# social-ai-uoft/sorrel

Measured on AMD Instinct MI355X. Metric: agent-steps/sec, higher is better.
Workload: dtype u8 grid, f32 obs

## Files before the change

### sorrel_amd/csrc/common.h

```cpp
#pragma once


constexpr int kBlock = 256;
constexpr int kWave = 64;
constexpr int kMaxPass = 2;

struct DevTables {
    uint32_t thr_lo[SGW_MAX_TYPES];
    uint32_t delta[4][SGW_MAX_TYPES];
    double value[SGW_MAX_TYPES];
    uint8_t spawn_choice[SGW_MAX_TYPES][SGW_MAX_CHOICES];
    uint8_t spawn_count[SGW_MAX_TYPES];
    uint8_t agent_type[SGW_MAX_AGENTS];
    uint8_t dense_choice[SGW_MAX_CHOICES];
    uint8_t layer_fill[8];
    uint8_t layer_border[8];
    uint8_t pad_[8];
    uint8_t rule[SGW_MAX_TYPES];
    int8_t rule_layer[SGW_MAX_TYPES];
    uint8_t rule_become[SGW_MAX_TYPES];
    uint8_t pad2_[SGW_MAX_TYPES];
    uint32_t rule_mask[SGW_MAX_TYPES];
    uint32_t delta3[SGW_MAX_TYPES];
    double appearance[SGW_MAX_TYPES][SGW_MAX_CHANNELS];
// ... 58 lines not shown
    uint32_t first_env;
    int64_t E;
    uint32_t epoch, turn, flags;
    int a0, a1;
    int do_move;
    int obs_post;
    int obs_u8;
    int agent_rule;
    uint32_t tag_it, tag_notit;
    double tag_reward;
    uint8_t* agent_state;
    uint8_t* agent_dir;
    int has_become;
    uint32_t quiet0, quiet1;
    uint32_t kind_pack;
    int beam_radius;
    uint32_t clean_beam, zap_beam, beam_block_mask;
    int total_factor;
    uint8_t* state_at_pov;
    uint64_t dense_thr;
    int dense_count;
    uint8_t* grid;
    uint8_t* pos;
    uint8_t* actions;
    float* obs;
    float* rewards;
    double* total;
    const DevTables* tab;
    const uint8_t* tmpl;
    int* status;
    int obs_stage;
    int stage_agents;
    int obs_next;
    int obs_A, obs_a0;
    int64_t obs_ag;
    int big_pitch;
    int big_stage;
    int big_stage_off;
    uint32_t* walk_ctr;
    int walk_word;
    int walk_static;
    int single_spawner;
    int rows_mode;
    int rows_by_agent;
    int onehot;
    int tail_kind, tail_len;
    const float* tail_table;
    const TurnState* ts;
    uint32_t nturns;
    int64_t ts_obs, ts_act, ts_rew;
    uint32_t extras;
    uint32_t drawn_mask;
    uint8_t* target_types;
};
constexpr uint32_t kExtraDrawn = 1u, kExtraTargets = 2u;
#ifdef SGW_JIT
constexpr bool kExtrasDefault = false;
#else
constexpr bool kExtrasDefault = true;
#endif
constexpr bool extras_default_tables(const int tc) { return kExtrasDefault && tc == 0; }
template <bool XTRAS>
__device__ __forceinline__ uint32_t extras_of(const Params& p) {
    if constexpr (XTRAS) return p.extras;
    else return 0u;
}

struct U4 {
    uint32_t x, y, z, w;
};

__device__ __forceinline__ uint32_t xor3(uint32_t a, uint32_t b, uint32_t k) {
    uint32_t d;
    asm("v_bitop3_b32 %0, %1, %2, %3 bitop3:0x96" : "=v"(d) : "v"(a), "v"(b), "s"(k));
    return d;
}

template <bool OWN_KEYS = true>
__device__ __forceinline__ U4 philox4x32_10(uint32_t c0, uint32_t c1, uint32_t c2, uint32_t c3,
                                            uint32_t k0, uint32_t k1) {
#ifndef SGW_DIAG_SHARED_KEYS
    if constexpr (OWN_KEYS) asm volatile("" : "+s"(k0), "+s"(k1));
#endif
#pragma unroll
    for (int r = 0; r < 10; ++r) {
        const uint64_t p0 = (uint64_t)0xD2511F53u * c0;
        const uint64_t p1 = (uint64_t)0xCD9E8D57u * c2;
        const uint32_t n0 = xor3((uint32_t)(p1 >> 32), c1, k0);
        const uint32_t n2 = xor3((uint32_t)(p0 >> 32), c3, k1);
        c1 = (uint32_t)p1;
        c3 = (uint32_t)p0;
        c0 = n0;
        c2 = n2;
        k0 += 0x9E3779B9u;
        k1 += 0xBB67AE85u;
    }
    return U4{c0, c1, c2, c3};
}

__device__ __forceinline__ uint32_t opaque(uint32_t v) {
    asm volatile("" : "+v"(v));
    return v;
}

struct PhiloxUniform {
    uint32_t r1_n2;
    uint32_t r2_n0;
    uint32_t r2_n2;
    uint32_t r3_n2;
};
__device__ __forceinline__ PhiloxUniform philox_uniform(const uint32_t c1, const uint32_t c2, const uint32_t c3, const uint32_t k0, const uint32_t k1) {
    const uint64_t p1 = (uint64_t)0xCD9E8D57u * c2;
    const uint32_t n0 = (uint32_t)(p1 >> 32) ^ c1 ^ k0;
    const uint64_t q0 = (uint64_t)0xD2511F53u * n0;
    PhiloxUniform u;
    u.r1_n2 = opaque(c3 ^ k1);
    u.r2_n0 = opaque((uint32_t)p1 ^ (k0 + 0x9E3779B9u));
    u.r2_n2 = opaque((uint32_t)(q0 >> 32) ^ (k1 + 0xBB67AE85u));
// ... 300 lines not shown
```

### sorrel_amd/csrc/plan.h

```cpp
#pragma once

struct Kernel {
    const void* host = nullptr;
    const char* host_name = "-";
    std::string want;
    bool x_twin = false;
    bool compile_time_tables = false;
    hipFunction_t jit = nullptr;
    hipFunction_t jit_x = nullptr;
    bool tried_x = false;
    bool tried = false;
    bool usable() const { return host != nullptr || !want.empty(); }
    const char* name() const { return (jit || (!host && !want.empty())) ? want.c_str() : host_name; }
};

uint64_t prob_threshold(double pr) {
    const double t = std::floor(pr * 4294967296.0);
    if (!(t > 0.0)) return 0;
    if (t >= 4294967296.0) return 4294967296ull;
    return (uint64_t)t;
}

int validate(const sgw_config* c) {
    if (!c) return fail(SGW_EINVAL, "config is NULL");
// ... 514 lines not shown
    p.fill_delta3 = h.delta3[c.fill_type];
    p.fill_delta16[0] = h.delta16[0][c.fill_type];
    p.fill_delta16[1] = h.delta16[1][c.fill_type];
    int& nspawn = w.nspawn;
    p.spawn_pat = 0xFFFFFFFFu;
    for (int t = 0; t < c.num_types; ++t) {
        if (c.type_rule[t] != SGW_RULE_SPAWN) continue;
        ++nspawn;
        p.spawn_pat = 0x01010101u * (uint32_t)t;
        const uint64_t thr = prob_threshold(c.spawn_prob[t]);
        p.spawn_thr = (uint32_t)(thr & 0xFFFFFFFFull);
        p.spawn_full = thr >= 4294967296ull ? 1u : 0u;
        p.spawn_n = c.spawn_count[t];
        p.choice_lo = p.choice_hi = 0;
        for (int k = 0; k < c.spawn_count[t]; ++k) {
            if (k < 4) p.choice_lo |= (uint32_t)c.spawn_choice[t][k] << (8 * k);
            else p.choice_hi |= (uint32_t)c.spawn_choice[t][k] << (8 * (k - 4));
        }
    }
    p.single_spawner = nspawn <= 1 ? 1 : 0;
    p.onehot = onehot ? 1 : 0;
    p.nturns = 1;
    p.obs_A = c.num_agents;
    p.obs_a0 = 0;
    p.seed_lo = (uint32_t)c.seed;
    p.seed_hi = (uint32_t)(c.seed >> 32);
    p.first_env = (uint32_t)c.first_env_id;
    p.E = c.num_envs;
    p.dense_thr = prob_threshold(c.dense_prob);
    p.dense_count = c.dense_count;
    p.obs_post = c.obs_post;
    p.agent_rule = c.agent_rule;
    p.tag_it = c.tag_it_type;
    p.tag_notit = c.tag_notit_type;
    p.tag_reward = c.tag_reward;
    p.agent_mask = 0;
    for (int a = 0; a < c.num_agents; ++a) p.agent_mask |= 1u << (c.agent_type[a] & 31u);
    if (c.agent_rule == SGW_AGENT_RULE_TAG) p.agent_mask |= (1u << (c.tag_it_type & 31u)) | (1u << (c.tag_notit_type & 31u));
    p.has_become = 0;
    p.become_mask = 0;
    for (int t = 0; t < c.num_types; ++t)
        if (c.type_rule[t] == SGW_RULE_BECOME_IF) {
            p.has_become = 1;
            p.become_mask |= 1u << t;
        }
    p.quiet0 = p.quiet1 = 0xFFFFFFFFu;
    for (int z = 0; z < c.layers; ++z) {
        const uint32_t t = c.layer_fill_type[z];
        if (t >= (uint32_t)c.num_types || c.type_rule[t] != SGW_RULE_NONE) continue;
        const uint32_t w = 0x01010101u * t;
        if (p.quiet0 == 0xFFFFFFFFu || p.quiet0 == w) p.quiet0 = w;
        else if (p.quiet1 == 0xFFFFFFFFu || p.quiet1 == w) p.quiet1 = w;
    }
    p.kind_pack = 0;
    for (int a = 0; a < c.num_actions; ++a) p.kind_pack |= (uint32_t)(c.action_kind[a] & 3u) << (2 * a);
    p.beam_radius = c.beam_radius;
    p.clean_beam = c.clean_beam_type;
    p.zap_beam = c.zap_beam_type;
    p.beam_block_mask = c.beam_block_mask;
    p.total_factor = c.reward_total_factor > 0 ? c.reward_total_factor : 1;
}

void plan_family(Planning& w, Plan* e) {
    PLANNING_INPUTS;
    const int nspawn = w.nspawn;
    const bool plain_move = c.agent_rule == SGW_AGENT_RULE_MOVE;
    const bool tagk = c.agent_rule == SGW_AGENT_RULE_TAG;
    const bool simple_rules = !p.has_become && c.agent_rule != SGW_AGENT_RULE_CLEANUP;
    const bool vec16 = (p.env_stride & 15) == 0 && p.env_stride >= p.cells_pad;
    const int rules_units = (c.num_envs >= 16384 || o.rules_11k) ? kMaxUnitsPlain : kMaxUnitsRules;
    bool rules_8k = !simple_rules && !tagk && vec16 && p.cells_pad > 4096 && (p.cells_pad >> 4) <= 64 * rules_units && p.VV <= 128;
    if (!o.fast_rules || o.force_generic) rules_8k = false;
    const bool fast_8k_ok = simple_rules && (onehot || (e->rgb16 && c.num_channels == 3)) && vec16 && nspawn <= 1 && p.cells_pad > 4096 && (p.cells_pad >> 4) <= 64 * kMaxUnitsPlain && p.VV <= 128;
    bool fast_8k = fast_8k_ok && c.num_envs >= (p.cells_pad <= 8192 ? 4096 : 16384);
    if (o.fast_8k == 0) fast_8k = false;
    if (o.fast_8k == 1) fast_8k = fast_8k_ok;
    if (o.force_generic) fast_8k = false;
    e->wpe = (p.cells_pad <= 4096 || rules_8k || fast_8k) ? 1 : 4;
    if (o.force_big && simple_rules && !o.force_generic) e->wpe = 4;
    const bool many_agents = c.num_agents > 64;
    if (many_agents) e->wpe = 4;
    const int epb = kBlock / (e->wpe * kWave);
    e->lds_bytes = (size_t)p.tab_bytes + (size_t)epb * p.env_lds;
    e->fast = e->wpe == 1 && vec16 && (p.cells_pad >> 4) <= 64 * (fast_8k ? kMaxUnitsPlain : kMaxUnits) && nspawn <= 1 && p.VV <= 128 && simple_rules;
    e->fast_rules = !e->fast && e->wpe == 1 && vec16 && (p.cells_pad >> 4) <= 64 * rules_units && p.VV <= 128 &&
                    !tagk && (p.cells_pad <= 4096 || rules_8k);
    if (!o.fast_rules) e->fast_rules = false;
    e->fast = e->fast || e->fast_rules;
    if (many_agents) e->fast = e->fast_rules = false;
    const bool rgb16_fast = e->rgb16 && e->fast && !e->fast_rules && c.num_channels == 3;
    const bool bytes_ok = onehot || rgb16_fast;
    e->fast_tab_bytes = bytes_ok ? 4 * SGW_MAX_TYPES * 4 : SGW_MAX_TYPES * SGW_MAX_CHANNELS * 8;
    bool agents_impassable = true;
    for (int a = 0; a < c.num_agents; ++a) agents_impassable = agents_impassable && !c.type_passable[c.agent_type[a]];
    const bool tag_move = tagk;
    e->big = e->wpe == 4 && vec16 && nspawn <= 1 && p.VV <= 128 && agents_impassable && (plain_move || tag_move) && simple_rules && !many_agents;
    e->big_threads = kBigThreads;
    if (e->big) e->big_threads = big_threads_for(o, onehot, c.num_agents, p.VV);
    w.plain_move = plain_move; w.tagk = tagk; w.many_agents = many_agents; w.fast_8k = fast_8k; w.epb = epb;
    w.rgb16_fast = rgb16_fast; w.bytes_ok = bytes_ok;
}

void plan_obs_staging(Planning& w, Plan* e) {
    PLANNING_INPUTS;
    const bool tagk = w.tagk, fast_8k = w.fast_8k, bytes_ok = w.bytes_ok;
    bool stage_kernel = false;
// ... 128 lines not shown
    if (e->whole_env_burst && static_map && !e->fast_rules && ((C * (2 * r + 1) * (2 * r + 1)) & 1) == 0) {
        if (L == 2 && C == 6 && r == 3 && H == 32 && W == 32 && !tagk) {
            e->k_sweep_rows.host = reinterpret_cast<const void*>(&step_fast_rows<2, 6, 3, 32, 32>);
            e->k_sweep_rows.host_name = "step_fast_rows<2, 6, 3, 32, 32>";
        }
        if (jit) e->k_sweep_rows.want = fast_rows_id(L, C, r, H, W, tagk);
        if (jit) e->k_sweep_rows_tail.want = fast_rows_id(L, C, r, H, W, tagk, true);
    }
    if (jit && !e->whole_env_burst && stage_kernel && e->onehot && !e->rgb16 && e->stage_agents >= 1) {
        e->k_sweep_rows.want = step.d.shaped(L, C, r, jh, jw).rowsx_id();
        e->sweep_rows_chunked = !e->k_sweep_rows.want.empty();
    }
}
void plan_instances(Planning& w, Plan* e) {
    PLANNING_INPUTS;
    const bool tagk = w.tagk, many_agents = w.many_agents;
    const bool tag_move = tagk;
    const int L = c.layers, C = c.num_channels, r = c.vision_radius, H = c.height, W = c.width;
    for (Kernel* k : {&e->k_step, &e->k_plain, &e->k_multi, &e->k_walk}) k->x_twin = true;
    e->k_sweep_rows.x_twin = !e->fast;
    if (e->fast) {
        plan_fast_instances(w, e);
    } else if (e->big) {
        set_prebuilt(e->k_step, pick_big(e->onehot, L, C, r, tag_move, e->big_threads));
        if (!tag_move) set_prebuilt(e->k_multi, pick_big_multi(e->onehot, L, C, r));
        if (!tag_move && ((p.cells + 15) >> 4) <= 4 * e->big_threads)
            set_prebuilt(e->k_walk, pick_big_walk(e->onehot, L, C, r, e->big_threads));
        if (jit) {
            e->k_sweep_rows.want = big_id(e->onehot, L, C, r, false, false, tag_move, e->big_threads, true);
            e->k_step.want = big_id(e->onehot, L, C, r, false, false, tag_move, e->big_threads);
            if (!tag_move) e->k_multi.want = big_id(e->onehot, L, C, r, true, false, false, kBigThreads);
            if (e->k_walk.host) e->k_walk.want = big_id(e->onehot, L, C, r, false, true, false, e->big_threads);
        }
    } else {
        if (many_agents) {
            e->k_step.host = pick_step_many(e->onehot, c.agent_rule, false, &e->k_step.host_name);
            e->k_multi.host = nullptr;
        } else {
            e->k_step.host = pick_step(o, e->group, e->onehot, L, C, c.agent_rule, r, H, W, false, &e->k_step.host_name);
            e->k_multi.host = pick_step(o, e->group, e->onehot, L, C, c.agent_rule, r, H, W, true, &e->k_multi.host_name);
        }
        if (jit) {
            e->k_step.want = generic_id(e->group, e->onehot, L, C, c.agent_rule, r, H, W, false, many_agents);
            e->k_multi.want = generic_id(e->group, e->onehot, L, C, c.agent_rule, r, H, W, true, many_agents);
            e->k_sweep_rows.want = generic_id(e->group, e->onehot, L, C, c.agent_rule, r, H, W, false, many_agents, true);
        }
    }
    if (!o.big_walk) e->k_walk = Kernel();
    for_each_kernel(*e, kHasPrebuiltTwin, [](Kernel& k) {
        if (k.host && k.want == k.host_name) k.want.clear();
        return 0;
    });
    e->multi_turn = e->k_multi.usable();
}

void plan_row_kernels(Planning& w, Plan* e) {
    PLANNING_INPUTS;
    const bool plain_move = w.plain_move;
    const int L = c.layers, C = c.num_channels, r = c.vision_radius;
    e->reset_fn = pick_reset(e->wpe);
    e->phase_ok = plain_move && e->wpe == 4;
    if (o.phase_kernel >= 0) e->phase_ok = plain_move && o.phase_kernel == 1;
    if (e->onehot && p.cells >= 8 && o.phase_rows) {
        const int NW = (C + 3) / 4;
        e->k_rows.x_twin = true;
        e->k_rows.host = pick_rows(L, NW, r, &e->k_rows.host_name, &e->k_obs_rows.host, &e->k_obs_rows.host_name);
        if (jit && !e->k_rows.host && r >= 1 && r <= 7) {
            e->k_rows.want = rows_id("phase_rows", L, NW, r);
            e->k_obs_rows.want = rows_id("observe_rows", L, NW, r);
        }
        if (!plain_move) e->k_rows = Kernel();
        if (e->k_obs_rows.usable()) {
            const int V = 2 * r + 1;
            e->rows_epb = e->rows_wpb = 4 * (64 / (V <= 4 ? 4 : (V <= 8 ? 8 : 16)));
            e->rows_lds = (size_t)4 * (NW * 34 * 4 + SGW_MAX_TYPES * 8 + (((e->rows_epb / 4) * C * V * V + 15) & ~15));
        }
    }
}

void plan_geometry(Planning& w, Plan* e) {
    PLANNING_INPUTS;
    const int epb = w.epb, epb_step = w.epb_step;
    p.stage_agents = e->stage_agents;
    if (o.fast_wg_per_cu > 0) { e->fast_wg_cap = o.fast_wg_per_cu; e->fast_wg_cap_forced = true; }
    e->grid_blocks = (int)ceil_div(p.E, (e->fast || e->big) ? epb : epb_step);
    if (e->k_walk.usable()) {
        const size_t walk_lds = e->step_lds_bytes - (size_t)(e->big_threads / 64) * e->big_stage;
        const int per_cu = resident_per_cu(e->big_threads, walk_lds, SGW_WALK_WAVES);
        const int plain_per_cu = resident_per_cu(e->big_threads, e->step_lds_bytes, SGW_BIG_WAVES);
        e->walk_blocks = per_cu * w.num_cus;
        e->walk_min_envs = (int64_t)plain_per_cu * w.num_cus * 3 / 2;
        e->walk_max_envs = e->big_stage ? (int64_t)plain_per_cu * w.num_cus * 9 / 4 : (int64_t)plain_per_cu * w.num_cus * 3;
        if (o.big_walk_blocks > 0) {
            e->walk_blocks = o.big_walk_blocks;
            e->walk_min_envs = e->walk_blocks;
            e->walk_max_envs = INT64_MAX;
        }
    }
    if (e->big) {
        const int64_t by_lds = (int64_t)(kLdsPerCu / (((e->step_lds_bytes + 1023) & ~(size_t)1023) + 1024));
        const int64_t resident = std::max<int64_t>(1, std::min<int64_t>(2048 / e->big_threads, by_lds));
        e->big_stage_min_envs = resident * w.num_cus * 7 / 4;
        if (o.big_stage == 1) e->big_stage_min_envs = 0;
    }
    e->reset_blocks = (int)ceil_div(p.E, epb);
}
// ... 21 lines not shown
```

### sorrel_amd/csrc/sgw.hip

```cpp
#include <hip/hip_runtime.h>
#include <hip/hiprtc.h>

#include <dlfcn.h>
#include <fcntl.h>
#include <sys/stat.h>
#include <unistd.h>

#include <algorithm>
#include <chrono>
#include <cmath>
#include <cstdarg>
#include <cstdio>
#include <cstdlib>
#include <cstring>
#include <mutex>
#include <new>
#include <string>
#include <unordered_map>
#include <vector>

#include "../../include/sgw.h"

namespace {

// ... 1299 lines not shown
    *launches = e->launches;
    e->ms_acc = 0.0;
    e->launches = 0;
    return SGW_OK;
}

int sgw_get_step_times_ms(sgw_engine* e, float* out_ms, int64_t capacity, int64_t* count) {
    if (!e || !count || (capacity > 0 && !out_ms)) return fail(SGW_EINVAL, "sgw_get_step_times_ms: NULL argument");
    if (int rc = time_drain(e)) return rc;
    const int64_t n = std::min<int64_t>((int64_t)e->series.size(), std::max<int64_t>(capacity, 0));
    for (int64_t i = 0; i < n; ++i) out_ms[i] = e->series[(size_t)i];
    const int64_t lost = (int64_t)e->series.size() - n + e->series_dropped;
    *count = n;
    e->series.clear();
    e->series_dropped = 0;
    if (lost > 0) {
        fail(SGW_OK, "sgw_get_step_times_ms: %lld launches not returned (capacity %lld, series cap %lld)", (long long)lost,
             (long long)capacity, (long long)kSeriesCap);
        return 1;
    }
    return SGW_OK;
}

int sgw_set_auto_reset(sgw_engine* e, uint32_t max_turns, double* episode_return) {
    if (!e) return fail(SGW_EINVAL, "sgw_set_auto_reset: NULL engine");
    e->auto_max_turns = max_turns;
    e->episode_return = max_turns ? episode_return : nullptr;
    return SGW_OK;
}

int sgw_set_wg_per_cu(sgw_engine* e, int wg_per_cu) {
    if (!e) return fail(SGW_EINVAL, "sgw_set_wg_per_cu: NULL engine");
    if (wg_per_cu < -1 || wg_per_cu > 8) return fail(SGW_EINVAL, "wg_per_cu must be -1 (never cap), 0 (automatic) or 1..8");
    e->wg_per_cu = wg_per_cu;
    return SGW_OK;
}

int sgw_launch_info(sgw_engine* e, char* buf, int64_t capacity) {
    if (!e || !buf || capacity < 1) return fail(SGW_EINVAL, "sgw_launch_info: NULL argument");
    Params p = e->base;
    p.a0 = 0; p.a1 = p.A; p.flags = SGW_STEP_SWEEP | SGW_STEP_RANDOM_ACTIONS; p.do_move = 1;
    p.obs = reinterpret_cast<float*>(16); p.obs_u8 = e->obs_format == SGW_OBS_U8 ? 1 : 0;
    StepLaunch d;
    if (int rc = step_launch(e, p, nullptr, &d)) return rc;
    Kernel& k = *d.k;
    if (d.walk) (void)resolve_kernel(e, k);
    int per_cu = 0;
    hipError_t oe = k.jit ? hipModuleOccupancyMaxActiveBlocksPerMultiprocessor(&per_cu, k.jit, (int)d.threads, d.lds_info)
                          : (k.host ? hipOccupancyMaxActiveBlocksPerMultiprocessor(&per_cu, k.host, (int)d.threads, d.lds_info) : hipErrorInvalidValue);
    if (oe != hipSuccess) per_cu = -1;
    const char* phase = e->k_rows.usable() ? e->k_rows.name() : (e->phase_ok ? (e->onehot ? "phase_kernel<true>" : "phase_kernel<false>") : "the step kernel");
    const char* srows = e->k_sweep_rows.usable() ? ((e->tail_kind != SGW_TAIL_NONE && e->fast && !e->sweep_rows_chunked && e->k_sweep_rows_tail.jit) ? e->k_sweep_rows_tail.name()
                                                                                                                                                   : e->k_sweep_rows.name()) : "-";
    snprintf(buf, (size_t)capacity, "%s group=%d threads=%d lds=%zu env_lds=%d obs_stage=%d stage_agents=%d grid=%d wg_per_cu=%d cap=%s%d phase=%s big_stage=%d specialised=%d sweep_rows=%s",
             k.name(),
             (e->fast || e->big) ? (e->big ? e->big_threads : e->wpe * kWave) : e->group,
             (int)d.threads, d.lds_info, e->step_env_lds, e->obs_stage, e->stage_agents,
             (int)d.blocks, per_cu,
             e->wg_per_cu == 0 ? "auto:" : (e->wg_per_cu < 0 ? "never:" : "forced:"), d.cap, phase, d.big_stage,
             k.jit ? 1 : 0, srows);
    return SGW_OK;
}

}
```

### sorrel_amd/csrc/step_fast.h

```cpp
#pragma once

constexpr int kMaxUnits = 4;
constexpr int kMaxUnitsRules = 8;
constexpr int kMaxUnitsPlain = 11;
constexpr size_t kLdsPerCu = 160 * 1024;
constexpr size_t kCacheResidentGrid = (size_t)288 << 20;

#define OBS_STORE(ptr, val) (*(ptr) = (val))


template <class Draw>
__device__ __forceinline__ uint32_t sweep_hits_with(const uint4& u, const Params& p, Draw draw) {
    uint32_t hits = 0;
    const uint32_t pat = p.spawn_pat & 0xFFu;
#pragma unroll
    for (int k = 0; k < 4; ++k) {
        const uint32_t dv = k == 0 ? u.x : k == 1 ? u.y : k == 2 ? u.z : u.w;
        const bool m0 = (dv & 0xFFu) == pat, m1 = ((dv >> 8) & 0xFFu) == pat, m2 = ((dv >> 16) & 0xFFu) == pat, m3 = (dv >> 24) == pat;
        if (m0 | m1 | m2 | m3) {
            const U4 w = draw(k);
            const bool f = p.spawn_full != 0;
            uint32_t hb = 0;
            hb |= (m0 && (f || w.x < p.spawn_thr)) ? 1u : 0u;
            hb |= (m1 && (f || w.y < p.spawn_thr)) ? 2u : 0u;
// ... 258 lines not shown
    const uint32_t vt_lo = (uint32_t)__double_as_longlong(vtab), vt_hi = (uint32_t)(__double_as_longlong(vtab) >> 32);
    const uint32_t vt_f32 = __float_as_uint((float)vtab);
    const bool write_obs = !(p.flags & SGW_STEP_NO_OBS);
    const bool do_sweep = (p.flags & SGW_STEP_SWEEP) != 0;
    const bool dirty = do_sweep || (p.do_move && p.a1 > p.a0);
    const bool sweep_only = !RULES && (MULTI ? p.nturns : 1u) == 1u && !(p.do_move && p.a1 > p.a0);

    {
        double tot = p.do_move ? p.total[env] : 0.0;

#ifdef SGW_STAMPS
        asm volatile("s_waitcnt vmcnt(0)" ::: "memory");
#endif
        STAMP(1);
        [[maybe_unused]] uint32_t hits[NU];
        if constexpr (!kStatic || ((TL * TH * TW) & 15) != 0) {
            if (cells & 15) {
#pragma unroll
                for (int k = 0; k < NU; ++k)
                    if (lane + 64 * k == nunits - 1) {
                        const int tail = cells & 15;
                        uint32_t d[4] = {u[k].x, u[k].y, u[k].z, u[k].w};
#pragma unroll
                        for (int q = 0; q < 4; ++q) {
                            const int keep = tail - 4 * q;
                            if (keep <= 0) d[q] = 0xFFFFFFFFu;
                            else if (keep < 4) d[q] |= 0xFFFFFFFFu << (8 * keep);
                        }
                        u[k] = make_uint4(d[0], d[1], d[2], d[3]);
                    }
            }
        }
#pragma unroll
        for (int k = 0; k < NU; ++k)
            if (lane + 64 * k < nunits) lg16[lane + 64 * k] = u[k];
        if constexpr (RULES || !kStatic) {
            const uint4* src = reinterpret_cast<const uint4*>(p.grid + env * p.env_stride);
            for (int i = 64 * NU + lane; i < nunits; i += 64) {
                uint4 v = src[i];
                if ((cells & 15) && i == nunits - 1) {
                    const int tail = cells & 15;
                    uint32_t d[4] = {v.x, v.y, v.z, v.w};
#pragma unroll
                    for (int q = 0; q < 4; ++q) {
                        const int keep = tail - 4 * q;
                        if (keep <= 0) d[q] = 0xFFFFFFFFu;
                        else if (keep < 4) d[q] |= 0xFFFFFFFFu << (8 * keep);
                    }
                    v = make_uint4(d[0], d[1], d[2], d[3]);
                }
                lg16[i] = v;
            }
        }
        int st_lane = 0;
        uint32_t taddr_v = 0xFFFFFFFFu, oaddr_v = 0, npos = 0, rew_bits = 0, moved = 0;
        const uint32_t nturns = MULTI ? p.nturns : 1u;
        for (uint32_t tix = 0; tix < nturns; ++tix) {
        const uint32_t turn = turn0 + tix;
        constexpr uint32_t kNotDrawn = 0xFFFFFFFFu;
        if (rnd) act = kNotDrawn;
        if constexpr (RULES) {
            gsync<1>();
            if (do_sweep) {
                sweep_ordered<1, 64>(p, rt, lg, env_id, lane, turn, ep4, L, HW);
            }
        } else if constexpr (!kStatic) {
            gsync<1>();
            if (do_sweep) {
                sweep_single<64>(p, lg, env_id, lane, turn, ep4,
                                 sweep_only ? reinterpret_cast<uint32_t*>(p.grid + env * p.env_stride) : nullptr);
                gsync<1>();
            }
        } else {
            if (tix > 0) {
                gsync<1>();
#pragma unroll
                for (int k = 0; k < NU; ++k)
                    if (lane + 64 * k < nunits) u[k] = lg16[lane + 64 * k];
            }
            const PhiloxUniform pu = philox_uniform(turn, env_id, ep4 | SGW_STREAM_SPAWN, p.seed_lo, p.seed_hi);
#pragma unroll
            for (int k = 0; k < NU; ++k) {
                hits[k] = 0;
                if ((k < kFullRounds || !kTailDword) && lane + 64 * k < nunits && do_sweep)
                    hits[k] = sweep_hits<kOwnKeys>(u[k], (uint32_t)(lane + 64 * k), p, pu);
            }
            gsync<1>();
            if (do_sweep) {
                typedef typename HitMask<(NU > 2)>::type hm_t;
                static_assert(NU <= 4, "16 hit bits per unit, four units per lane");
                hm_t hm = 0;
#pragma unroll
                for (int k = 0; k < NU; ++k) hm |= (hm_t)hits[k] << (16 * k);
                auto unit_off = [&](const uint32_t b) { return ((uint32_t)lane + 64u * (b >> 4)) * 16u + (b & 15u); };
                auto kind_of = [&](const uint32_t pick) { return (uint8_t)(((pick < 4 ? p.choice_lo : p.choice_hi) >> (8 * (pick & 3u))) & 0xFFu); };
                uint32_t nlist = 0;
                bool fused = false;
                if constexpr (!ROWS && !MULTI) {
                    uint32_t fl = p.flags;
                    asm("" : "+s"(fl));
                    if (stage && !(fl & SGW_STEP_NO_OBS) && p.do_move && rnd && p.a0 == 0 && p.a1 == p.A && p.obs_stage >= 256) {
                        uint16_t* list = reinterpret_cast<uint16_t*>(ob);
                        const uint32_t room = 64u - (uint32_t)p.A;
                        hm_t rest = hm;
                        uint64_t m = __ballot(rest != 0);
                        while (m != 0 && nlist <= room) {
// ... 104 lines not shown
            const int i0 = (lo + 3) >> 2, i1 = he >> 2;
            const int ie = lane == 0 ? i0 - 1 : i1;
            const bool edge = lane == 0 ? (lo & 3) != 0 : (lane == 1 && (he & 3) != 0 && (i1 >= i0 || (lo & 3) == 0));
            if (ROWX || !p.obs_u8) {
                float* gb = ROWX ? row_dst - sh : p.obs + (e0 - sh);
                burst_emit<true>(gb, i0, i1, lane, [&](const int i) { return ob4[i]; }, tof);
                if (edge) {
                    const uint32_t b = ob4[ie];
#pragma unroll
                    for (int j = 0; j < 4; ++j)
                        if (4 * ie + j >= lo && 4 * ie + j < he) gb[4 * ie + j] = tof((b >> (8 * j)) & 0xFFu);
                }
            } else {
                uint8_t* gb = reinterpret_cast<uint8_t*>(p.obs) + (e0 - sh);
                burst_emit<false>(gb, i0, i1, lane, [&](const int i) { return ob4[i]; }, tof);
                if (edge) {
                    const uint32_t b = ob4[ie];
#pragma unroll
                    for (int j = 0; j < 4; ++j)
                        if (4 * ie + j >= lo && 4 * ie + j < he) gb[4 * ie + j] = (uint8_t)(b >> (8 * j));
                }
            }
            if constexpr (ROWX) {
                if (p.tail_kind != SGW_TAIL_NONE) {
                    float* t = row_dst + C * VV;
                    if (p.tail_kind == SGW_TAIL_AGENT_IS_IT) {
                        const uint32_t ty_ = (uint32_t)__builtin_amdgcn_readlane((int)atype, a_lo);
                        if (lane == 0) t[0] = ty_ == p.tag_it ? 1.f : 0.f;
                    } else {
                        const int ay_ = __builtin_amdgcn_readlane((int)(yx & 0xFFu), a_lo), ax_ = __builtin_amdgcn_readlane((int)(yx >> 8), a_lo);
                        const float* src = p.tail_table + ((int64_t)ay_ * W + ax_) * p.tail_len;
                        for (int k = lane; k < p.tail_len; k += 64) t[k] = src[k];
                    }
                }
            }
            if (!last) {
                uint8_t t = 0;
                if (lane < hi - he) t = ob[he + lane];
                gsync<1>();
                if (lane < hi - he) ob[lane] = t;
                ch_shift = (uint32_t)(hi - he);
                ch_lo = 0;
            }
            gsync<1>();
        };
        [[maybe_unused]] uint32_t fill_v[NW];
        constexpr bool kFillRegs = ONEHOT && kStatic && !RULES && !STAGE && !P3 && !I16;
        if constexpr (kFillRegs) {
#pragma unroll
            for (int q = 0; q < NW; ++q) fill_v[q] = opaque(p.fill_delta[q]);
        }
        constexpr bool kVersioned = ONEHOT && kStatic && !kStageAlways && !TAG && !RULES && !ROWS && !MULTI;
        const bool lean = kVersioned && stage && write_obs && !p.obs_next;
        auto window = [&](const int a, const int y, const int x, const int s_o, auto lean_c) {
            constexpr bool LEAN = decltype(lean_c)::value;
            {
                const int cbase = s_o - zoff;
                int a_s = a;
                if constexpr (kVersioned && !LEAN) asm volatile("" : "+s"(a_s));
                [[maybe_unused]] float* obase = p.obs + turn_obs + ((env * p.obs_A + (a_s - p.obs_a0)) * (int64_t)C) * VV;
#pragma unroll
                for (int k = 0; k < 2; ++k) {
                    if (64 * k >= VV) break;
                    const int w = lane + 64 * k;
                    if (w < VV) {
#ifdef SGW_DIAG_SKIP_GATHER
                        if (p.turn != 0xFFFFFFFFu) continue;
#endif
                        const bool inb = (unsigned)(y + wdi[k]) < (unsigned)H && (unsigned)(x + wdj[k]) < (unsigned)W;
                        const int off = inb ? cbase + woff[k] : 0;
                        [[maybe_unused]] float* o = obase + w;
                        if constexpr (ONEHOT) {
                            uint32_t cnt[NW];
#pragma unroll
                            for (int q = 0; q < NW; ++q) cnt[q] = 0;
#pragma unroll
                            for (int z = 0; z < (TL ? TL : 1); ++z) {
                                const uint32_t t = lg[z * HW + off] & 31u;
#pragma unroll
                                for (int q = 0; q < NW; ++q) cnt[q] += wdelta[q * 32 + t];
                            }
                            if constexpr (TL == 0) {
                                for (int z = 1; z < L; ++z) {
                                    const uint32_t t = lg[z * HW + off] & 31u;
#pragma unroll
                                    for (int q = 0; q < NW; ++q) cnt[q] += wdelta[q * 32 + t];
                                }
                            }
#pragma unroll
                            for (int q = 0; q < NW; ++q) cnt[q] = inb ? cnt[q] : (kFillRegs ? fill_v[q] : P3 ? p.fill_delta3 : I16 ? p.fill_delta16[q] : p.fill_delta[q]);
                            auto chan = [&](const int c) -> uint32_t {
                                if constexpr (P3) return (cnt[0] >> (3 * c)) & 7u;
                                else if constexpr (I16) return min((cnt[c >> 1] >> (16 * (c & 1))) & 0xFFFFu, 255u);
                                else return (cnt[c >> 2] >> (8 * (c & 3))) & 0xFFu;
                            };
                            if (LEAN || stage) {
                                uint8_t* os = ob + (kStageAlways ? (int)ch_shift + ((a - ch_a0) * C) * VV : (a * C) * VV) + w;
                                if constexpr (TC != 0) {
#pragma unroll
                                    for (int c = 0; c < CMAX; ++c)
                                        if (c < C) os[c * VV] = (uint8_t)chan(c);
                                } else {
#pragma unroll
                                    for (int g = 0; g < (CMAX + 3) / 4; ++g)
                                        if (4 * g < C) {
#pragma unroll
                                            for (int b = 0; b < 4; ++b)
                                                if (4 * g + b < CMAX) os[(4 * g + b) * VV] = (uint8_t)chan(4 * g + b);
                                        }
                                }
                            } else if constexpr (kStageAlways) {
                            } else if (!p.obs_u8) {
#pragma unroll
                                for (int c = 0; c < CMAX; ++c)
                                    if (c < C) OBS_STORE(o + c * VV, tof(chan(c)));
                            } else {
                                uint8_t* o8 = reinterpret_cast<uint8_t*>(p.obs) + (o - p.obs);
#pragma unroll
                                for (int c = 0; c < CMAX; ++c)
                                    if (c < C) o8[c * VV] = (uint8_t)chan(c);
                            }
                        } else {
                            for (int c = 0; c < C; ++c) {
                                double acc = wapp[lg[off] & 31u][c];
                                for (int z = 1; z < L; ++z) acc += wapp[lg[z * HW + off] & 31u][c];
                                OBS_STORE(o + c * VV, obs_finish(inb ? acc : wapp[p.fill_type][c], p.obs_post));
                            }
                        }
                    }
                }
            }
        };
        const int a_end = (p.obs_next && p.a1 < p.A) ? p.a1 + 1 : p.a1;
        for (int a = p.a0; a < a_end; ++a) {
            if constexpr (ROWX) {
                if (a > p.a0 && write_obs) emit_chunk(a - 1, a, true);
                ch_a0 = a;
                row_dst = static_cast<float*>(rp->p[a]) + env * rp->stride;
                ch_lo = ch_shift = (uint32_t)(reinterpret_cast<uintptr_t>(row_dst) >> 2) & kLineMask;
            } else if constexpr (kStageAlways) {
                if (a - ch_a0 == p.stage_agents) {
                    if (write_obs) emit_chunk(ch_a0, a, false);
                    ch_a0 = a;
                }
            }
            const uint32_t yx_a = (uint32_t)__builtin_amdgcn_readlane((int)yx, a);
            const int y = (int)(yx_a & 0xFFu), x = (int)(yx_a >> 8);
            const int s_o = zoff + y * W + x;
            if (lean) {
                if constexpr (kVersioned) window(a, y, x, s_o, BoolC<true>{});
            } else if (p.obs_next ? a == p.a1 : write_obs) {
                window(a, y, x, s_o, BoolC<false>{});
            }
            if (!p.do_move || a >= p.a1) continue;
            const uint32_t s_t = (uint32_t)__builtin_amdgcn_readlane((int)taddr_v, a);
            const uint32_t my_type = (uint32_t)__builtin_amdgcn_readlane((int)atype, a);
            const bool valid = s_t != 0xFFFFFFFFu;
            if constexpr (RULES) {
                if (p.agent_rule == SGW_AGENT_RULE_CLEANUP) {
                    const uint32_t kd = (uint32_t)__builtin_amdgcn_readlane((int)kind_v, a);
                    const uint32_t kind = kd & 3u, ndir = kd >> 4;
                    const bool aok = (kd & 4u) != 0;
                    const uint32_t facing = (uint32_t)__builtin_amdgcn_readlane((int)adir, a) & 3u;
                    const int ay = __builtin_amdgcn_readlane((int)py, a), ax = __builtin_amdgcn_readlane((int)px, a);
                    if (aok && kind != SGW_ACTION_MOVE && p.zA + 1 < L) {
                        if (lane < 3 * p.beam_radius) {
                            const int arm = lane / p.beam_radius, i = lane - arm * p.beam_radius;
                            const int fy = facing == 0 ? -1 : facing == 2 ? 1 : 0, fx = facing == 1 ? 1 : facing == 3 ? -1 : 0;
                            const int ry = facing == 1 ? 1 : facing == 3 ? -1 : 0, rx = facing == 0 ? 1 : facing == 2 ? -1 : 0;
                            const int step = arm == 0 ? i + 1 : i, side = arm == 0 ? 0 : (arm == 1 ? 1 : -1);
                            const int by = ay + side * ry + step * fy, bx = ax + side * rx + step * fx;
                            if ((unsigned)by < (unsigned)H && (unsigned)bx < (unsigned)W) {
                                const int boff = (p.zA + 1) * HW + by * W + bx;
                                if (!((p.beam_block_mask >> (lg[boff] & 31u)) & 1u))
                                    lg[boff] = (uint8_t)(kind == SGW_ACTION_CLEAN ? p.clean_beam : p.zap_beam);
                            }
                        }
                        gsync<1>();
                    }
                    double val = 0.0;
                    uint32_t t = 0xFFu;
                    if (valid) {
                        const int tc = (int)s_t - zoff;
                        for (int zl = 0; zl < L; ++zl) {
                            const uint32_t tz = (uint32_t)__builtin_amdgcn_readfirstlane((int)lg[zl * HW + tc]) & 31u;
                            const uint32_t lo_ = (uint32_t)__builtin_amdgcn_readlane((int)vt_lo, (int)tz);
                            const uint32_t hi_ = (uint32_t)__builtin_amdgcn_readlane((int)vt_hi, (int)tz);
                            val += __longlong_as_double(((long long)hi_ << 32) | lo_);
                        }
                        t = (uint32_t)__builtin_amdgcn_readfirstlane((int)lg[s_t]);
                    }
                    const bool pass = valid && t < (uint32_t)p.T && ((p.pass_mask >> (t & 31u)) & 1u);
                    if (pass && lane == 0) {
                        lg[s_t] = (uint8_t)my_type;
                        lg[s_o] = (uint8_t)p.default_type;
                    }
                    moved = lane == a ? (pass ? 1u : 0u) : moved;
                    adir = (lane == a && aok && kind == SGW_ACTION_MOVE && ndir < 4u) ? ndir : adir;
                    rew_bits = lane == a ? __float_as_uint((float)val) : rew_bits;
                    tot += val * (double)(p.total_factor - 1);
                    tot += val;
                    gsync<1>();
                    continue;
                }
            }
            const uint32_t t = (uint32_t)__builtin_amdgcn_readfirstlane((int)lg[valid ? s_t : (uint32_t)s_o]);
// ... 171 lines not shown
```

Measured before the change: 4.766 billion.

## Skip gathering inert uniform layers in onehot observation window

At plan time, layers whose fill type never changes, is never spawned, and contributes zero to every observation channel are marked inert. In the kernel, each wave checks via ballot whether such a layer is still uniformly filled and, if so, skips that layer's per-cell lookups when building observation windows. Interior agents also skip per-cell bounds checks, and the lean and non-lean window paths are merged into one lambda. This adds a per-step uniformity scan and more code complexity, and relies on the inert analysis being correct.

```diff
diff --git a/sorrel_amd/csrc/common.h b/sorrel_amd/csrc/common.h
--- a/sorrel_amd/csrc/common.h
+++ b/sorrel_amd/csrc/common.h
@@ -134,6 +134,7 @@
     uint32_t extras;
     uint32_t drawn_mask;
     uint8_t* target_types;
+    uint32_t inert_layers, inert_fill;
 };
 constexpr uint32_t kExtraDrawn = 1u, kExtraTargets = 2u;
 #ifdef SGW_JIT
@@ -146,6 +147,14 @@
 __device__ __forceinline__ uint32_t extras_of(const Params& p) {
     if constexpr (XTRAS) return p.extras;
     else return 0u;
+}
+
+__device__ __forceinline__ uint32_t unit_differs(const uint4 u, const uint32_t k) {
+    uint32_t d;
+    asm("v_bitop3_b32 %0, %1, %2, %3 bitop3:0x7e" : "=v"(d) : "v"(u.x), "v"(u.y), "s"(k));
+    asm("v_bitop3_b32 %0, %1, %2, %3 bitop3:0xf6" : "=v"(d) : "v"(d), "v"(u.z), "s"(k));
+    asm("v_bitop3_b32 %0, %1, %2, %3 bitop3:0xf6" : "=v"(d) : "v"(d), "v"(u.w), "s"(k));
+    return d;
 }
 
 struct U4 {
diff --git a/sorrel_amd/csrc/plan.h b/sorrel_amd/csrc/plan.h
--- a/sorrel_amd/csrc/plan.h
+++ b/sorrel_amd/csrc/plan.h
@@ -590,6 +590,26 @@
         if (p.quiet0 == 0xFFFFFFFFu || p.quiet0 == w) p.quiet0 = w;
         else if (p.quiet1 == 0xFFFFFFFFu || p.quiet1 == w) p.quiet1 = w;
     }
+    p.inert_layers = p.inert_fill = 0;
+    if (onehot && c.agent_rule == SGW_AGENT_RULE_MOVE && !p.has_become) {
+        uint32_t produced = 0;
+        for (int t = 0; t < c.num_types; ++t) {
+            if (c.type_rule[t] == SGW_RULE_SPAWN)
+                for (int k = 0; k < c.spawn_count[t] && k < SGW_MAX_CHOICES; ++k) produced |= 1u << (c.spawn_choice[t][k] & 31u);
+            if (c.type_rule[t] == SGW_RULE_BECOME_IF) produced |= 1u << (c.rule_become[t] & 31u);
+        }
+        for (int z = 0; z < c.layers && z < 4; ++z) {
+            const uint32_t t = c.layer_fill_type[z];
+            if (z == c.agent_layer || t >= (uint32_t)c.num_types) continue;
+            if (c.type_rule[t] != SGW_RULE_NONE || ((produced | p.drawn_mask) >> t) & 1u) continue;
+            bool zero = h.delta3[t] == 0;
+            for (int q = 0; q < 4; ++q) zero = zero && h.delta[q][t] == 0;
+            for (int k = 0; k < c.num_channels; ++k) zero = zero && c.appearance[t][k] == 0.0;
+            if (!zero) continue;
+            p.inert_layers |= 1u << z;
+            p.inert_fill |= t << (8 * z);
+        }
+    }
     p.kind_pack = 0;
     for (int a = 0; a < c.num_actions; ++a) p.kind_pack |= (uint32_t)(c.action_kind[a] & 3u) << (2 * a);
     p.beam_radius = c.beam_radius;
@@ -824,6 +844,7 @@
         return 0;
     });
     e->multi_turn = e->k_multi.usable();
+    if (!e->fast || e->fast_rules || tagk || e->rgb16) p.inert_layers = p.inert_fill = 0;
 }
 
 void plan_row_kernels(Planning& w, Plan* e) {
diff --git a/sorrel_amd/csrc/sgw.hip b/sorrel_amd/csrc/sgw.hip
--- a/sorrel_amd/csrc/sgw.hip
+++ b/sorrel_amd/csrc/sgw.hip
@@ -1375,14 +1375,14 @@
     const char* phase = e->k_rows.usable() ? e->k_rows.name() : (e->phase_ok ? (e->onehot ? "phase_kernel<true>" : "phase_kernel<false>") : "the step kernel");
     const char* srows = e->k_sweep_rows.usable() ? ((e->tail_kind != SGW_TAIL_NONE && e->fast && !e->sweep_rows_chunked && e->k_sweep_rows_tail.jit) ? e->k_sweep_rows_tail.name()
                                                                                                                                                    : e->k_sweep_rows.name()) : "-";
-    snprintf(buf, (size_t)capacity, "%s group=%d threads=%d lds=%zu env_lds=%d obs_stage=%d stage_agents=%d grid=%d wg_per_cu=%d cap=%s%d phase=%s big_stage=%d specialised=%d sweep_rows=%s",
+    snprintf(buf, (size_t)capacity, "%s group=%d threads=%d lds=%zu env_lds=%d obs_stage=%d stage_agents=%d grid=%d wg_per_cu=%d cap=%s%d phase=%s big_stage=%d specialised=%d sweep_rows=%s inert_layers=0x%x",
              k.name(),
              (e->fast || e->big) ? (e->big ? e->big_threads : e->wpe * kWave) : e->group,
              (int)d.threads, d.lds_info, e->step_env_lds, e->obs_stage, e->stage_agents,
              (int)d.blocks, per_cu,
              e->wg_per_cu == 0 ? "auto:" : (e->wg_per_cu < 0 ? "never:" : "forced:"), d.cap, phase, d.big_stage,
-             k.jit ? 1 : 0, srows);
-    return SGW_OK;
-}
-
-}
+             k.jit ? 1 : 0, srows, e->base.inert_layers);
+    return SGW_OK;
+}
+
+}
diff --git a/sorrel_amd/csrc/step_fast.h b/sorrel_amd/csrc/step_fast.h
--- a/sorrel_amd/csrc/step_fast.h
+++ b/sorrel_amd/csrc/step_fast.h
@@ -334,6 +334,34 @@
                 lg16[i] = v;
             }
         }
+        constexpr bool kGather = ONEHOT && kStatic && !TAG && !RULES && !STAGE && !MULTI && !P3 && !I16;
+        [[maybe_unused]] uint32_t gskip = 0;
+        if constexpr (kGather && TL > 1 && ((TH * TW) & 15) == 0) {
+            const uint32_t cand = p.inert_layers;
+            if (cand != 0) {
+                uint32_t inert = 0;
+#pragma unroll
+                for (int z = 0; z < (TL < 4 ? TL : 4); ++z) {
+                    if (!((cand >> z) & 1u)) continue;
+                    const uint32_t pat = ((p.inert_fill >> (8 * z)) & 0xFFu) * 0x01010101u;
+                    const int lo = z * (TH * TW / 16), hi = lo + TH * TW / 16;
+                    bool foreign = false;
+#pragma unroll
+                    for (int k = 0; k < NU; ++k) {
+                        if (64 * k >= hi || 64 * k + 64 <= lo) continue;
+                        const bool here = lane + 64 * k >= lo && lane + 64 * k < hi;
+                        foreign = foreign | (here & (unit_differs(u[k], pat) != 0));
+                    }
+                    inert |= (__ballot(foreign) == 0 ? 1u : 0u) << z;
+                }
+#pragma unroll
+                for (int j = 1; j < TL; ++j) {
+                    const int z = p.zA + j >= TL ? p.zA + j - TL : p.zA + j;
+                    gskip |= ((inert >> z) & 1u) << j;
+                }
+            }
+            asm volatile("" : "+s"(gskip));
+        }
         int st_lane = 0;
         uint32_t taddr_v = 0xFFFFFFFFu, oaddr_v = 0, npos = 0, rew_bits = 0, moved = 0;
         const uint32_t nturns = MULTI ? p.nturns : 1u;
@@ -544,13 +572,12 @@
         }
         constexpr bool kVersioned = ONEHOT && kStatic && !kStageAlways && !TAG && !RULES && !ROWS && !MULTI;
         const bool lean = kVersioned && stage && write_obs && !p.obs_next;
-        auto window = [&](const int a, const int y, const int x, const int s_o, auto lean_c) {
-            constexpr bool LEAN = decltype(lean_c)::value;
+        auto window = [&](const int a, const int y, const int x, const int s_o) {
             {
-                const int cbase = s_o - zoff;
-                int a_s = a;
-                if constexpr (kVersioned && !LEAN) asm volatile("" : "+s"(a_s));
-                [[maybe_unused]] float* obase = p.obs + turn_obs + ((env * p.obs_A + (a_s - p.obs_a0)) * (int64_t)C) * VV;
+                [[maybe_unused]] const int cbase = s_o - zoff;
+                [[maybe_unused]] const bool interior = kGather && H > 2 * r && W > 2 * r && (unsigned)(y - r) < (unsigned)(H - 2 * r) && (unsigned)(x - r) < (unsigned)(W - 2 * r);
+                auto obs_base = [&](const int a_s) { return p.obs + turn_obs + ((env * p.obs_A + (a_s - p.obs_a0)) * (int64_t)C) * VV; };
+                [[maybe_unused]] float* obase = kVersioned ? nullptr : obs_base(a);
 #pragma unroll
                 for (int k = 0; k < 2; ++k) {
                     if (64 * k >= VV) break;
@@ -559,34 +586,70 @@
 #ifdef SGW_DIAG_SKIP_GATHER
                         if (p.turn != 0xFFFFFFFFu) continue;
 #endif
-                        const bool inb = (unsigned)(y + wdi[k]) < (unsigned)H && (unsigned)(x + wdj[k]) < (unsigned)W;
-                        const int off = inb ? cbase + woff[k] : 0;
+                        [[maybe_unused]] bool inb = true;
+                        [[maybe_unused]] int off = 0;
+                        if constexpr (!kGather) {
+                            inb = (unsigned)(y + wdi[k]) < (unsigned)H && (unsigned)(x + wdj[k]) < (unsigned)W;
+                            off = inb ? cbase + woff[k] : 0;
+                        }
                         [[maybe_unused]] float* o = obase + w;
                         if constexpr (ONEHOT) {
                             uint32_t cnt[NW];
-#pragma unroll
-                            for (int q = 0; q < NW; ++q) cnt[q] = 0;
-#pragma unroll
-                            for (int z = 0; z < (TL ? TL : 1); ++z) {
-                                const uint32_t t = lg[z * HW + off] & 31u;
-#pragma unroll
-                                for (int q = 0; q < NW; ++q) cnt[q] += wdelta[q * 32 + t];
-                            }
-                            if constexpr (TL == 0) {
-                                for (int z = 1; z < L; ++z) {
+                            if constexpr (kGather) {
+                                const uint8_t* ca = (lg + s_o) + woff[k];
+                                if (!interior) {
+                                    inb = (unsigned)(y + wdi[k]) < (unsigned)H && (unsigned)(x + wdj[k]) < (unsigned)W;
+                                    int zo = zoff;
+                                    asm volatile("" : "+s"(zo));
+                                    ca = inb ? ca : lg + zo;
+                                }
+                                {
+                                    const uint32_t t = *ca & 31u;
+#pragma unroll
+                                    for (int q = 0; q < NW; ++q) cnt[q] = wdelta[q * 32 + t];
+                                }
+#pragma unroll
+                                for (int j = 1; j < TL; ++j) {
+                                    if (!((gskip >> j) & 1u)) {
+                                        int zo = zoff;
+                                        asm volatile("" : "+s"(zo));
+                                        const int dz = (zo + j * HW >= TL * HW ? j - TL : j) * HW;
+                                        const uint32_t t = ca[dz] & 31u;
+#pragma unroll
+                                        for (int q = 0; q < NW; ++q) cnt[q] += wdelta[q * 32 + t];
+                                        asm volatile("" : "+v"(cnt[0]));
+                                    }
+                                }
+                                if (!interior) {
+#pragma unroll
+                                    for (int q = 0; q < NW; ++q) cnt[q] = inb ? cnt[q] : fill_v[q];
+                                    asm volatile("" : "+v"(cnt[0]));
+                                }
+                            } else {
+#pragma unroll
+                                for (int q = 0; q < NW; ++q) cnt[q] = 0;
+#pragma unroll
+                                for (int z = 0; z < (TL ? TL : 1); ++z) {
                                     const uint32_t t = lg[z * HW + off] & 31u;
 #pragma unroll
                                     for (int q = 0; q < NW; ++q) cnt[q] += wdelta[q * 32 + t];
                                 }
+                                if constexpr (TL == 0) {
+                                    for (int z = 1; z < L; ++z) {
+                                        const uint32_t t = lg[z * HW + off] & 31u;
+#pragma unroll
+                                        for (int q = 0; q < NW; ++q) cnt[q] += wdelta[q * 32 + t];
+                                    }
+                                }
+#pragma unroll
+                                for (int q = 0; q < NW; ++q) cnt[q] = inb ? cnt[q] : (kFillRegs ? fill_v[q] : P3 ? p.fill_delta3 : I16 ? p.fill_delta16[q] : p.fill_delta[q]);
                             }
-#pragma unroll
-                            for (int q = 0; q < NW; ++q) cnt[q] = inb ? cnt[q] : (kFillRegs ? fill_v[q] : P3 ? p.fill_delta3 : I16 ? p.fill_delta16[q] : p.fill_delta[q]);
                             auto chan = [&](const int c) -> uint32_t {
                                 if constexpr (P3) return (cnt[0] >> (3 * c)) & 7u;
                                 else if constexpr (I16) return min((cnt[c >> 1] >> (16 * (c & 1))) & 0xFFFFu, 255u);
                                 else return (cnt[c >> 2] >> (8 * (c & 3))) & 0xFFu;
                             };
-                            if (LEAN || stage) {
+                            if (kVersioned ? lean : stage) {
                                 uint8_t* os = ob + (kStageAlways ? (int)ch_shift + ((a - ch_a0) * C) * VV : (a * C) * VV) + w;
                                 if constexpr (TC != 0) {
 #pragma unroll
@@ -602,15 +665,22 @@
                                         }
                                 }
                             } else if constexpr (kStageAlways) {
-                            } else if (!p.obs_u8) {
-#pragma unroll
-                                for (int c = 0; c < CMAX; ++c)
-                                    if (c < C) OBS_STORE(o + c * VV, tof(chan(c)));
                             } else {
-                                uint8_t* o8 = reinterpret_cast<uint8_t*>(p.obs) + (o - p.obs);
-#pragma unroll
-                                for (int c = 0; c < CMAX; ++c)
-                                    if (c < C) o8[c * VV] = (uint8_t)chan(c);
+                                if constexpr (kVersioned) {
+                                    int a_s = a;
+                                    asm volatile("" : "+s"(a_s));
+                                    o = obs_base(a_s) + w;
+                                }
+                                if (!p.obs_u8) {
+#pragma unroll
+                                    for (int c = 0; c < CMAX; ++c)
+                                        if (c < C) OBS_STORE(o + c * VV, tof(chan(c)));
+                                } else {
+                                    uint8_t* o8 = reinterpret_cast<uint8_t*>(p.obs) + (o - p.obs);
+#pragma unroll
+                                    for (int c = 0; c < CMAX; ++c)
+                                        if (c < C) o8[c * VV] = (uint8_t)chan(c);
+                                }
                             }
                         } else {
                             for (int c = 0; c < C; ++c) {
@@ -639,11 +709,7 @@
             const uint32_t yx_a = (uint32_t)__builtin_amdgcn_readlane((int)yx, a);
             const int y = (int)(yx_a & 0xFFu), x = (int)(yx_a >> 8);
             const int s_o = zoff + y * W + x;
-            if (lean) {
-                if constexpr (kVersioned) window(a, y, x, s_o, BoolC<true>{});
-            } else if (p.obs_next ? a == p.a1 : write_obs) {
-                window(a, y, x, s_o, BoolC<false>{});
-            }
+            if (lean || (p.obs_next ? a == p.a1 : write_obs)) window(a, y, x, s_o);
             if (!p.do_move || a >= p.a1) continue;
             const uint32_t s_t = (uint32_t)__builtin_amdgcn_readlane((int)taddr_v, a);
             const uint32_t my_type = (uint32_t)__builtin_amdgcn_readlane((int)atype, a);
```

Result: slower. 4.558 billion (-4.4%).
